# water-chika/ray-tracing-gpu-vulkan

Measured on AMD Instinct MI355X. Metric: Msamples/s (1920x1080 RTIOW scene, depth 50), higher is better.
Workload: dtype f32; 1 GPU; rtiow-1920x1080-10000spp-depth50 (BASELINE config 3 workload); width=1920, height=1080, spp=10000, depth=50, spheres=488, accel=grid-lds-rec, walk=uniform grid (3D DDA) staged in LDS, with the winner's gate and shading records, structure_build=host (binned-SAH LBVH + uniform grid), uploaded per frame, rng=hash, sample_chunks=10, parallelism=1 GPU, frames_in_flight=1

## Files before the change

ray-tracing-gpu-vulkan_amd/csrc/rt_internal.h:

```cpp
#pragma once

#include <stdint.h>

#include "../../include/rt_abi.h"
#include "rt_hand_out.h"

namespace rt {

struct alignas(16) GeomRec {
    float cx, cy, cz, rr;
};

struct alignas(16) MatRec {
    float c0x, c0y, c0z, attr;
    float c1x, c1y, c1z;
    uint32_t type_tex;
};
constexpr uint32_t kMatDielConst = 1u << 16;

#if defined(__HIPCC__)
__host__ __device__
#endif
inline bool colours_in_unit(const Sphere& s) {
    auto in = [](float v) { return v >= 0.0f && v <= 1.0f; };
// ... 17 lines not shown
        m.c1x = ef;
        m.c1y = qf * qf;
        m.c1z = qb * qb;
        m.type_tex |= kMatDielConst;
    }
    return m;
}

struct alignas(16) BvhNode {
    float lox, loy, loz;
    uint32_t escape;
    float hix, hiy, hiz;
    uint32_t first_count;
};

struct GridInfo {
    float gmin[3];
    float gmax[3];
    float cs[3];
    float inv_cs[3];
    float margin;
    float lo_m[3];
    float hi_m[3];
    uint32_t n[3];
    uint32_t n_cells, n_refs;
};

#ifndef RT_TRACE_BLOCK
#define RT_TRACE_BLOCK 768
#endif
constexpr unsigned kLaneSumLdsBytes = 3u * 8u * RT_TRACE_BLOCK;
constexpr unsigned kCoopLdsBytes = (2u * 16u + 8u + 4u) * RT_TRACE_BLOCK;
constexpr unsigned kCqLdsBytes = (128u * 4u + 4u) * (RT_TRACE_BLOCK / 64u) + 8u * RT_TRACE_BLOCK;
constexpr unsigned kBatchQueue = 64u;
constexpr unsigned kBatchLdsBytes = (4u + 16u + 16u + 12u) * RT_TRACE_BLOCK;
constexpr uint32_t kBatchMaxDepth = 1u << 26;

struct DeviceScene {
    uint32_t n_spheres = 0;
    GeomRec* geom = nullptr;
    float* radius = nullptr;
    MatRec* mat = nullptr;
    uint32_t n_big = 0;
    uint32_t* big_ids = nullptr;
    uint32_t n_nodes = 0;
    BvhNode* nodes = nullptr;
    BvhNode* nodes_raw = nullptr;
    GeomRec* leaf_geom = nullptr;
    uint32_t* leaf_ids = nullptr;
    uint32_t n_leaf = 0;
    BvhNode* nodes_oct = nullptr;
    float* treelet = nullptr;
    uint32_t* treelet_count = nullptr;
    float small_rmax = 0.0f;
    float small_rmin = 0.0f;
    GridInfo grid{};
    uint32_t* cell_start = nullptr;
    GeomRec* grid_rec = nullptr;
    uint32_t* grid_ids = nullptr;
};

enum : uint32_t { ACCEL_BRUTE = 1, ACCEL_LBVH_GLOBAL = 2, ACCEL_LBVH_LDS = 3, ACCEL_LBVH_OCT = 4,
                  ACCEL_LBVH_TOP = 5, ACCEL_GRID = 6, ACCEL_GRID_GLOBAL = 7, ACCEL_GRID_COOP = 8,
                  ACCEL_GRID_GLOBAL_COOP = 9, ACCEL_GRID_REC = 10, ACCEL_GRID_CQ = 11, ACCEL_GRID_REC_CQ = 12,
                  ACCEL_COUNT = 13 };

enum : int { MODE_STREAM = 0, MODE_HASH = 1, MODE_PROBE = 2, MODE_FEATURES = 3, MODE_SCATTER = 4 };

// ... 73 lines not shown
    const GeomRec* grid_rec;
    const uint32_t* grid_ids;
    float* accum;
    uint32_t* out;
    unsigned long long* fixed;
    Counters* counters;
    const float* big_tab;
    const BlockEntry* block_tab;
    const TabSize* tab_size;
    const float* probe_rays;
    uint32_t* probe_out;
    float* feat0;
    float* feat1;
};

struct ScatterProbeParams {
    uint32_t n_spheres;
    const GeomRec* geom;
    const float* radius;
    const MatRec* mat;
    uint32_t n;
    const float* rays;
    const uint32_t* ids;
    const float* t;
    const uint32_t* seeds;
    uint32_t* out;
};

constexpr int kFixedFracBits = 24;
constexpr uint32_t kFixedFlush = 128;

constexpr uint32_t kBigMax = 64;
constexpr uint32_t kRecStatic = 512;
constexpr uint32_t kNoRowsLds = 0xffffffffu;
constexpr uint32_t kHashMaxSpp = 1u << 19;

}
```

ray-tracing-gpu-vulkan_amd/csrc/rt_kernels.hip:

```cpp
#include <hip/hip_runtime.h>

#include "rt_device_math.h"
#include "rt_internal.h"
#include "rt_launchers.h"
#include "rt_trace_diag.h"
#include "rt_trace_prims.h"
#include "rt_trace_units.h"
#include "rt_trace_shade.h"
#include "rt_trace_walk.h"
#include "rt_trace_grid_coop.h"
#include "rt_trace_batch.h"

using namespace rtd;

namespace {

#ifndef RT_BRUTE_WAVES_PER_SIMD
#define RT_BRUTE_WAVES_PER_SIMD 6
#endif
#ifndef RT_TRACE_WAVES_PER_SIMD
#define RT_TRACE_WAVES_PER_SIMD 6
#endif
constexpr uint32_t kBruteBlock = 256;
constexpr uint32_t kTraceBlock = RT_TRACE_BLOCK;
// ... 256 lines not shown
        const uint32_t n = min(P.n_spheres, rt::kRecStatic);
        for (uint32_t i = threadIdx.x; i < n; i += kTraceBlock) {
            const rt::GeomRec g = P.geom[i];
            s_rec[3 * i] = make_float4(g.cx, g.cy, g.cz, P.radius[i]);
            s_rec[3 * i + 1] = mat4[2 * i];
            s_rec[3 * i + 2] = mat4[2 * i + 1];
        }
        __syncthreads();
        lbvh_loop<COUNT, CQ ? LAYOUT_GRID_CQ : LAYOUT_GRID, MODE, true, FLAT, TAB>(P, reinterpret_cast<const float4*>(cst), lds,
                                                                              ids, s_rec, s_rec);
        return;
    }
    __syncthreads();
    lbvh_loop<COUNT, COOP ? LAYOUT_GRID_COOP : CQ ? LAYOUT_GRID_CQ : LAYOUT_GRID, MODE, false, FLAT, TAB>(P, reinterpret_cast<const float4*>(cst), lds, ids,
                                        reinterpret_cast<const float4*>(P.geom),
                                        reinterpret_cast<const float4*>(P.mat));
}

template <bool FLAT>
__global__ __launch_bounds__(kTraceBlock, RT_TRACE_WAVES_PER_SIMD) void rt_trace_grid_batch_kernel(const rt::TraceParams P) {
    UTIL_INIT;
    PLACEMENT_RECORD(P);
    extern __shared__ float4 lds[];
    const uint32_t nr = P.grid.n_refs, nc1 = P.grid.n_cells + 1u;
    const uint32_t n_id4 = (nr + 3u) / 4u;
    const float4* rec = reinterpret_cast<const float4*>(P.grid_rec);
    for (uint32_t i = threadIdx.x; i < nr; i += kTraceBlock) lds[i] = rec[i];
    uint32_t* ids = reinterpret_cast<uint32_t*>(lds + nr);
    for (uint32_t i = threadIdx.x; i < nr; i += kTraceBlock) ids[i] = P.grid_ids[i];
    uint32_t* cst = reinterpret_cast<uint32_t*>(lds + nr + n_id4);
    for (uint32_t i = threadIdx.x; i < nc1; i += kTraceBlock) cst[i] = P.cell_start[i];
    stage_walk_params(P, threadIdx.x);
    stage_rows(P, threadIdx.x, kTraceBlock);
    __syncthreads();
    batch_loop<FLAT>(P, reinterpret_cast<const float4*>(cst), lds, ids, reinterpret_cast<const float4*>(P.geom),
                     reinterpret_cast<const float4*>(P.mat));
    UTIL_FLUSH;
}

template <bool COUNT, int MODE, int TAB = 0>
__global__ __launch_bounds__(kTraceBlock, RT_TRACE_WAVES_PER_SIMD) void rt_trace_top_kernel(const rt::TraceParams P) {
    UTIL_INIT;
    PLACEMENT_RECORD(P);
    extern __shared__ float4 lds[];
    typedef const __attribute__((address_space(3))) float4* LdsF4;
    const uint32_t lbase = uint32_t(reinterpret_cast<uintptr_t>((LdsF4)lds));
    const uint32_t n_top = min(*P.treelet_count, rt::kTreeletCap);
    for (uint32_t i = threadIdx.x; i < n_top; i += kTraceBlock) {
        const float4* tl = reinterpret_cast<const float4*>(P.treelet);
        const float4 A = tl[2 * i], B = tl[2 * i + 1];
        const uint32_t miss = __float_as_uint(B.z), hit = __float_as_uint(B.w);
        lds[2 * i] = A;
        lds[2 * i + 1] = make_float4(B.x, B.y, __uint_as_float(miss == END ? END : lbase + miss * 32u),
                                     __uint_as_float(int32_t(hit) >= 0 ? lbase + hit * 32u : hit));
    }
    stage_walk_params(P, threadIdx.x);
    stage_rows(P, threadIdx.x, kTraceBlock);
    __syncthreads();
    lbvh_loop<COUNT, LAYOUT_TOP, MODE, false, false, TAB>(P, lds, reinterpret_cast<const float4*>(P.leaf_geom), P.leaf_ids,
                                       reinterpret_cast<const float4*>(P.geom),
                                       reinterpret_cast<const float4*>(P.mat));
}

}

namespace rt {
// ... 89 lines not shown
```

ray-tracing-gpu-vulkan_amd/csrc/rt_trace_batch.h:

```cpp
#pragma once

#include <hip/hip_runtime.h>
#include <stdint.h>

#include "rt_device_math.h"
#include "rt_internal.h"
#include "rt_trace_grid.h"
#include "rt_trace_prims.h"
#include "rt_trace_shade.h"
#include "rt_trace_units.h"
#include "rt_trace_walk.h"

using namespace rtd;

namespace {

__shared__ uint32_t s_pix_chain[RT_TRACE_BLOCK];
__shared__ float4 s_q_o[RT_TRACE_BLOCK];
__shared__ float4 s_q_d[RT_TRACE_BLOCK];
__shared__ float s_q_thr[3 * RT_TRACE_BLOCK];
static_assert(rt::kBatchQueue == 64u, "one queue slot per lane of a wave: slot = wave0 + entry");
static_assert(sizeof(s_pix_chain) + sizeof(s_q_o) + sizeof(s_q_d) + sizeof(s_q_thr) == rt::kBatchLdsBytes,
              "rt_internal.h");

__device__ __forceinline__ void batch_path_end(uint32_t wave0, uint32_t pix, const Path& t, uint32_t segs) {
    unsigned long long* s = s_lane_sum + wave0 + pix;
    __hip_atomic_fetch_add(s, (unsigned long long)t.qx, __ATOMIC_RELAXED, __HIP_MEMORY_SCOPE_WAVEFRONT);
    __hip_atomic_fetch_add(s + RT_TRACE_BLOCK, (unsigned long long)t.qy, __ATOMIC_RELAXED, __HIP_MEMORY_SCOPE_WAVEFRONT);
    __hip_atomic_fetch_add(s + 2 * RT_TRACE_BLOCK, (unsigned long long)t.qz, __ATOMIC_RELAXED,
                           __HIP_MEMORY_SCOPE_WAVEFRONT);
    __hip_atomic_fetch_add(s_pix_chain + wave0 + pix, segs, __ATOMIC_RELAXED, __HIP_MEMORY_SCOPE_WAVEFRONT);
}

template <bool FLAT>
__device__ __forceinline__ bool batch_segment(const rt::TraceParams& P, const Camera& cam,
                                              const float4* __restrict__ cst, const float4* __restrict__ refs,
                                              const uint32_t* __restrict__ ids, const float4* __restrict__ geom4,
                                              const float4* __restrict__ mat4, uint32_t lane, bool active, Ray& r,
                                              Path& t) {
    uint32_t n_box = 0, n_sph = 0, n_empty = 0;
    __builtin_amdgcn_s_setprio(1);
    setup_ray<false>(P, r);
    r.walk = true;
    if (active) walk<false, LAYOUT_GRID, FLAT>(P, cst, refs, ids, r, n_box, n_sph, n_empty);
    HitRec hr{};
    float rad = 0.0f;
    if (active && r.bi != 0xffffffffu) {
        hr = load_hit(geom4, mat4, r.bi);
        rad = P.radius[r.bi];
    }
    unsigned long long regate =
        __ballot(active && r.bi != 0xffffffffu && !aabb_hit(hr.g.x, hr.g.y, hr.g.z, rad, r.o, r.inv));
    if (P.force_regate) regate = __ballot(active);
    if (__builtin_expect(regate != 0ull, 0)) {
        regate_brute<false>(P, geom4, lane, regate, r);
        if (((regate >> lane) & 1ull) && r.bi != 0xffffffffu) hr = load_hit(geom4, mat4, r.bi);
    }
    __builtin_amdgcn_s_setprio(0);
    bool more = false, fresh = false;
    if (active) {
        t.s = 0u;
        t.s_end = 1u;
        t.qx = t.qy = t.qz = 0u;
        more = shade_rec<rt::MODE_HASH, true, true>(P, cam, hr, t, r.bi, r.best, r.o, r.d, fresh);
    }
    return more;
}

template <bool FLAT>
__device__ __forceinline__ void batch_loop(const rt::TraceParams& P, const float4* __restrict__ cst,
                                           const float4* __restrict__ refs, const uint32_t* __restrict__ ids,
                                           const float4* __restrict__ geom4, const float4* __restrict__ mat4) {
    const uint32_t lane = lane_id();
    const uint32_t wave0 = __builtin_amdgcn_readfirstlane(threadIdx.x & ~63u);
    const Camera cam = load_camera(P);
    {
        unsigned long long* z = s_lane_sum + wave0 + lane;
        z[0] = z[RT_TRACE_BLOCK] = z[2 * RT_TRACE_BLOCK] = 0ull;
        s_pix_chain[wave0 + lane] = 0u;
        lane_order();
    }
    uint32_t seg_w = 0, smp_w = 0;
    WaveBlock blk;
    first_block<0>(P, lane, blk);
    if (lane == 0) atomicMin(&P.counters->t_first, __builtin_amdgcn_s_memrealtime());
    bool have = blk.end != blk.next;
    auto take = [&]() -> bool {
        if (blk.dry) return false;
        uint32_t nb = 0u;
        if (lane == 0) nb = atomicAdd(&P.counters->work_head, 64u);
        nb = __builtin_amdgcn_readfirstlane(nb);
        if (nb >= P.n_units) {
            blk.dry = true;
            if (lane == 0) atomicMin(&P.counters->t_dry, __builtin_amdgcn_s_memrealtime());
            return false;
        }
        take_block(P, lane, blk, nb >> 6, block_tile(P, nb >> 6));
        return true;
    };
    if (!have) have = take();
    uint32_t s = blk.s0, qn = 0u, px = 0u, word = 0u;
    bool valid = false, live = false;
    Ray r{};
    r.d = v3(0.0f, 0.0f, 1.0f);
    Path t{};
    auto block_pixels = [&]() {
        const uint32_t lx = (blk.tile % P.tiles_x) * 8u + (lane & 7u);
        const uint32_t ly = (blk.tile / P.tiles_x) * 8u + (lane >> 3);
        valid = lx < P.band_w && ly < P.band_h;
        px = lx | (ly << 16);
        s = blk.s0;
    };
    if (have) block_pixels();
    while (have) {
        const unsigned long long idle = __ballot(!live);
        if (idle && qn) {
            const uint32_t n = min(uint32_t(__popcll(idle)), qn);
            const uint32_t rank = __builtin_amdgcn_mbcnt_hi(uint32_t(idle >> 32), __builtin_amdgcn_mbcnt_lo(uint32_t(idle), 0u));
            if (!live && rank < n) {
                const uint32_t e = wave0 + (qn - 1u - rank);
                const float4 a = s_q_o[e], b = s_q_d[e];
                r.o = v3(a.x, a.y, a.z);
                r.d = v3(b.x, b.y, b.z);
                t.seed = __float_as_uint(a.w);
                word = __float_as_uint(b.w);
                t.thr = v3(s_q_thr[e], s_q_thr[RT_TRACE_BLOCK + e], s_q_thr[2 * RT_TRACE_BLOCK + e]);
                live = true;
            }
            qn -= n;
            lane_order();
        }
        const unsigned long long tracing = __ballot(live);
        if (~tracing != 0ull && s < blk.s1) {
            Path c{};
            Ray rc{};
            rc.d = v3(0.0f, 0.0f, 1.0f);
            if (valid) {
                c.px = px;
                c.pixel_seed = blk.seed;
                c.s = s;
                V3 v;
                camera_ray<rt::MODE_HASH, true>(P, cam, c, rc.o, v);
                rc.d = normalize(v);
            }
            const bool more = batch_segment<FLAT>(P, cam, cst, refs, ids, geom4, mat4, lane, valid, rc, c);
            const uint32_t n_valid = __popcll(__ballot(valid));
            seg_w += n_valid;
            smp_w += n_valid;
            if (valid && !more) batch_path_end(wave0, lane, c, 1u);
            const unsigned long long surv = __ballot(valid && more);
            if (valid && more) {
                const uint32_t e = wave0 + __builtin_amdgcn_mbcnt_hi(uint32_t(surv >> 32), __builtin_amdgcn_mbcnt_lo(uint32_t(surv), 0u));
                s_q_o[e] = make_float4(rc.o.x, rc.o.y, rc.o.z, __uint_as_float(c.seed));
                s_q_d[e] = make_float4(rc.d.x, rc.d.y, rc.d.z, __uint_as_float(lane | (c.depth << 6)));
                s_q_thr[e] = c.thr.x;
                s_q_thr[RT_TRACE_BLOCK + e] = c.thr.y;
                s_q_thr[2 * RT_TRACE_BLOCK + e] = c.thr.z;
            }
            qn = __popcll(surv);
            lane_order();
            s++;
            continue;
        }
        if (!tracing) {
            lane_order();
            unsigned long long* z = s_lane_sum + wave0 + lane;
            const unsigned long long x = z[0], y = z[RT_TRACE_BLOCK], w = z[2 * RT_TRACE_BLOCK];
            const uint32_t chain = s_pix_chain[wave0 + lane];
            z[0] = z[RT_TRACE_BLOCK] = z[2 * RT_TRACE_BLOCK] = 0ull;
            s_pix_chain[wave0 + lane] = 0u;
            lane_order();
            if (valid) {
                Path f{};
                f.px = px;
                f.segs = chain;
                if (x | y | w) add_fixed(P, f, x, y, w);
                record_tile_cost<rt::MODE_HASH>(P, f);
            }
            have = take();
            if (have) block_pixels();
            continue;
        }
        seg_w += __popcll(tracing);
        t.depth = word >> 6;
        const bool more = batch_segment<FLAT>(P, cam, cst, refs, ids, geom4, mat4, lane, live, r, t);
        if (live) {
            if (more) {
                word = (word & 63u) | (t.depth << 6);
            } else {
                batch_path_end(wave0, word & 63u, t, (word >> 6) + 1u);
                live = false;
            }
        }
    }
    if (lane == 0) {
        atomicAdd(&P.counters->segments, (unsigned long long)seg_w);
        atomicAdd(&P.counters->samples, (unsigned long long)smp_w);
        atomicMax(&P.counters->t_last, __builtin_amdgcn_s_memrealtime());
    }
}

}
```

ray-tracing-gpu-vulkan_amd/csrc/rt_trace_grid.h:

```cpp
#pragma once

#include <hip/hip_runtime.h>
#include <stdint.h>

#include "rt_device_math.h"
#include "rt_internal.h"
#include "rt_trace_diag.h"
#include "rt_trace_prims.h"

using namespace rtd;

namespace {

template <bool COUNT, bool PAIRS, bool FLAT = false>
__device__ __forceinline__ void grid_walk(const rt::TraceParams& P, const uint32_t* __restrict__ cstart,
                                          const float4* __restrict__ rec, const uint32_t* __restrict__ ids,
                                          Ray& r, uint32_t& n_cell, uint32_t& n_sph, uint32_t& n_empty) {
    const float4 ex = s_walk_entry[0], ey = s_walk_entry[1], ez = s_walk_entry[2];
    const float4 axx = s_walk_axis[0], axy = s_walk_axis[1], axz = s_walk_axis[2];
    const float lo0 = ex.x, lo1 = ey.x, lo2 = ez.x, hi0 = ex.y, hi1 = ey.y, hi2 = ez.y;
    const float ics[3] = {ex.z, ey.z, ez.z}, gmn[3] = {axx.y, axy.y, axz.y}, csz[3] = {axx.x, axy.x, axz.x};
    const int nm1[3] = {int(__float_as_uint(ex.w)), int(__float_as_uint(ey.w)), int(__float_as_uint(ez.w))};
    const uint32_t n0 = __float_as_uint(axx.w), n1 = __float_as_uint(axy.w);
    const float x0 = (lo0 - r.o.x) * r.inv.x, x1 = (hi0 - r.o.x) * r.inv.x;
    const float y0 = (lo1 - r.o.y) * r.inv.y, y1 = (hi1 - r.o.y) * r.inv.y;
    const float z0 = (lo2 - r.o.z) * r.inv.z, z1 = (hi2 - r.o.z) * r.inv.z;
    const float tn = fmaxf(fmaxf(fmaxf(fminf(x0, x1), fminf(y0, y1)), fminf(z0, z1)), T_MIN);
    const float tf = fminf(fminf(fminf(fmaxf(x0, x1), fmaxf(y0, y1)), fmaxf(z0, z1)), r.limit);
    if (!(tn <= tf)) return;
    auto cell_of = [&](float p, int k) {
        const int c = int(floorf((p - gmn[k]) * ics[k]));
        return min(max(c, 0), nm1[k]);
    };
    int cx = cell_of(__builtin_fmaf(tn, r.d.x, r.o.x), 0);
    int cy = FLAT ? 0 : cell_of(__builtin_fmaf(tn, r.d.y, r.o.y), 1);
    int cz = cell_of(__builtin_fmaf(tn, r.d.z, r.o.z), 2);
    const int sx = r.d.x > 0.0f ? 1 : (r.d.x < 0.0f ? -1 : 0);
    const int sy = r.d.y > 0.0f ? 1 : (r.d.y < 0.0f ? -1 : 0);
    const int sz = r.d.z > 0.0f ? 1 : (r.d.z < 0.0f ? -1 : 0);
    auto bound_t = [&](int c, int s, int k, float o, float inv) {
        const float plane = __builtin_fmaf(float(c + (s > 0 ? 1 : 0)), csz[k], gmn[k]);
        return s == 0 ? __builtin_inff() : (plane - o) * inv;
    };
    float tx = bound_t(cx, sx, 0, r.o.x, r.inv.x);
    float ty = bound_t(cy, sy, 1, r.o.y, r.inv.y);
    float tz = bound_t(cz, sz, 2, r.o.z, r.inv.z);
    uint32_t cell = FLAT ? uint32_t(cz) * n0 + uint32_t(cx) : (uint32_t(cz) * n1 + uint32_t(cy)) * n0 + uint32_t(cx);
    if constexpr (FLAT && PAIRS) {
        uint32_t b = cstart[cell], e = cstart[cell + 1];
        for (;;) {
            const float tm = fminf(fminf(tx, ty), tz);
            uint32_t ncell = cell;
            const bool more = dda_step_xz(tm, tx, ty, tz, cx, cz, sx, sz, ncell, r.o, r.inv);
            const uint32_t nb = cstart[ncell], ne = cstart[ncell + 1];
            if (COUNT) {
                n_cell++;
                n_empty += b == e ? 1u : 0u;
            }
            uint32_t j = b;
// ... 79 lines not shown
```

ray-tracing-gpu-vulkan_amd/csrc/rt_trace_prims.h:

```cpp
#pragma once

#include <hip/hip_runtime.h>
#include <stdint.h>

#include "rt_device_math.h"
#include "rt_internal.h"
#include "rt_trace_diag.h"

using namespace rtd;

namespace {

constexpr float T_MIN = 0.001f;
constexpr float T_MAX_SUCC = 0x1.388002p+13f;

__device__ __forceinline__ bool aabb_hit(float cx, float cy, float cz, float r, V3 o, V3 inv) {
    const float x0 = ((cx - r) - o.x) * inv.x, x1 = ((cx + r) - o.x) * inv.x;
    const float y0 = ((cy - r) - o.y) * inv.y, y1 = ((cy + r) - o.y) * inv.y;
    const float z0 = ((cz - r) - o.z) * inv.z, z1 = ((cz + r) - o.z) * inv.z;
    const float tnear = fmaxf(fmaxf(fmaxf(fminf(x0, x1), fminf(y0, y1)), fminf(z0, z1)), T_MIN);
    const float tfar = fminf(fminf(fminf(fmaxf(x0, x1), fmaxf(y0, y1)), fmaxf(z0, z1)), 10000.0f);
    return tnear <= tfar;
}

// ... 8 lines not shown
    if (D >= 0.0f) {
        const float sq = sqrt_cr(D);
        const float t1 = (-b - sq) * ia;
        const float t2 = (-b + sq) * ia;
        const float t = (t1 >= T_MIN) ? t1 : t2;
        if (t >= T_MIN && t < best && (!GATE || aabb_hit(cx, cy, cz, radius[id], o, inv))) {
            best = t;
            bi = id;
        }
    }
}

__device__ __forceinline__ bool behind(float b, float c) { return b >= 0x1p-60f && c >= 0.0f; }

typedef float f4v __attribute__((ext_vector_type(4)));
__device__ __forceinline__ float4 lds_reload(const float4* p) {
    const f4v v = *(const volatile __attribute__((address_space(3))) f4v*)(p);
    return make_float4(v.x, v.y, v.z, v.w);
}

__shared__ float4 s_walk_axis[3];
__shared__ float2 s_walk_slack;
__shared__ float4 s_walk_entry[3];
__device__ __forceinline__ void stage_walk_params(const rt::TraceParams& P, uint32_t tid) {
    if (tid < 3u) {
        const uint32_t stride = tid == 0u ? 1u : tid == 1u ? P.grid.n[0] : P.grid.n[0] * P.grid.n[1];
        s_walk_axis[tid] = make_float4(P.grid.cs[tid], P.grid.gmin[tid], __uint_as_float(stride),
                                       __uint_as_float(P.grid.n[tid]));
        s_walk_entry[tid] = make_float4(P.grid.lo_m[tid], P.grid.hi_m[tid], P.grid.inv_cs[tid],
                                        __uint_as_float(P.grid.n[tid] - 1u));
    }
    if (tid == 3u) s_walk_slack = make_float2(P.cull_near_abs, P.cull_abs);
}

__device__ __forceinline__ bool dda_step(float tm, float& tx, float& ty, float& tz, int& cx, int& cy, int& cz,
                                         int sx, int sy, int sz, uint32_t& cell, V3 o, V3 inv) {
    const bool mx = tx == tm, my = !mx && ty == tm, mz = !mx && !my;
    const float4 ax = s_walk_axis[mx ? 0 : my ? 1 : 2];
    const int s = mx ? sx : my ? sy : sz;
    const int c = (mx ? cx : my ? cy : cz) + s;
    if (uint32_t(c) >= __float_as_uint(ax.w)) return false;
    cx = mx ? c : cx;
    cy = my ? c : cy;
    cz = mz ? c : cz;
    cell = s > 0 ? cell + __float_as_uint(ax.z) : cell - __float_as_uint(ax.z);
    const float ok = mx ? o.x : my ? o.y : o.z, ik = mx ? inv.x : my ? inv.y : inv.z;
    const float tnew = (__builtin_fmaf(float(c + (s > 0 ? 1 : 0)), ax.x, ax.y) - ok) * ik;
    tx = mx ? tnew : tx;
    ty = my ? tnew : ty;
    tz = mz ? tnew : tz;
    return true;
}

__device__ __forceinline__ bool dda_step_xz(float tm, float& tx, float ty, float& tz, int& cx, int& cz, int sx,
                                            int sz, uint32_t& cell, V3 o, V3 inv) {
    const bool mx = tx == tm;
    if (!mx && ty == tm) return false;
    const float4 ax = s_walk_axis[mx ? 0 : 2];
    const int s = mx ? sx : sz;
    const int c = (mx ? cx : cz) + s;
    if (uint32_t(c) >= __float_as_uint(ax.w)) return false;
    cx = mx ? c : cx;
    cz = mx ? cz : c;
    cell = s > 0 ? cell + __float_as_uint(ax.z) : cell - __float_as_uint(ax.z);
    const float ok = mx ? o.x : o.z, ik = mx ? inv.x : inv.z;
    const float tnew = (__builtin_fmaf(float(c + (s > 0 ? 1 : 0)), ax.x, ax.y) - ok) * ik;
// ... 118 lines not shown
```

ray-tracing-gpu-vulkan_amd/csrc/rt_trace_shade.h:

```cpp
#pragma once

#include <hip/hip_runtime.h>
#include <stdint.h>

#include "rt_device_math.h"
#include "rt_internal.h"
#include "rt_trace_diag.h"
#include "rt_trace_units.h"

using namespace rtd;

namespace {

struct Camera { V3 lf, hor, ver, ulc, cup, crt; };

__device__ __forceinline__ Camera load_camera(const rt::TraceParams& P) {
    return Camera{v3(P.lf[0], P.lf[1], P.lf[2]), v3(P.hor[0], P.hor[1], P.hor[2]),
                  v3(P.ver[0], P.ver[1], P.ver[2]), v3(P.ulc[0], P.ulc[1], P.ulc[2]),
                  v3(P.cup[0], P.cup[1], P.cup[2]), v3(P.crt[0], P.crt[1], P.crt[2])};
}

template <int MODE, bool FAST = false>
__device__ __forceinline__ void camera_ray(const rt::TraceParams& P, const Camera& cam, Path& ps, V3& o, V3& v) {
    UTIL(7, true);
// ... 56 lines not shown
    d = normalize(v);
    return true;
}

template <int MODE, bool LSUM>
__device__ __forceinline__ void sample_end(const rt::TraceParams& P, Path& ps, const V3 col) {
    ps.s++;
    if (MODE == rt::MODE_HASH) {
        ps.qx += sample_fixed(col.x);
        ps.qy += sample_fixed(col.y);
        ps.qz += sample_fixed(col.z);
        if ((ps.s & (rt::kFixedFlush - 1u)) == 0u) flush_fixed<LSUM>(P, ps);
    } else {
        ps.sx += double(col.x);
        ps.sy += double(col.y);
        ps.sz += double(col.z);
    }
}

struct HitRec {
    float4 g, m0, m1;
};

__device__ __forceinline__ HitRec load_hit(const float4* __restrict__ geom4, const float4* __restrict__ mat4,
                                           uint32_t bi) {
    return HitRec{geom4[bi], mat4[2 * bi], mat4[2 * bi + 1]};
}

__shared__ float4 s_rec[3 * rt::kRecStatic];
__device__ __forceinline__ HitRec load_hit_rec(uint32_t bi) {
    return HitRec{s_rec[3 * bi], s_rec[3 * bi + 1], s_rec[3 * bi + 2]};
}

template <int MODE, bool LSUM, bool FAST = false>
__device__ __forceinline__ bool shade_rec(const rt::TraceParams& P, const Camera& cam, const HitRec& hr, Path& ps,
                                          uint32_t bi, float best, V3& o, V3& d, bool& fresh) {
    if constexpr (MODE == rt::MODE_PROBE) {
        const size_t i = size_t(ps.px >> 16) * P.band_w + (ps.px & 0xffffu);
        P.probe_out[2 * i] = bi;
        P.probe_out[2 * i + 1] = __float_as_uint(best);
        return false;
    }
    if constexpr (MODE == rt::MODE_FEATURES) {
        V3 alb = v3(0.7f, 0.8f, 1.0f), n = v3(0.0f, 0.0f, 0.0f);
        float depth = 0.0f, hit = 0.0f;
        if (bi != 0xffffffffu) {
            const V3 p = v3(__builtin_fmaf(best, d.x, o.x), __builtin_fmaf(best, d.y, o.y),
                            __builtin_fmaf(best, d.z, o.z));
            const float4 m0 = hr.m0, m1 = hr.m1;
            const uint32_t ttype = (__float_as_uint(m1.w) >> 8) & 0xffu;
            const V3 outward = normalize(sub(p, v3(hr.g.x, hr.g.y, hr.g.z)));
            const bool front = dot(d, outward) < 0.0f;
            n = front ? outward : neg(outward);
            alb = v3(m0.x, m0.y, m0.z);
            if (ttype == 1u && !checker_positive(p.x, p.y, p.z)) alb = v3(m1.x, m1.y, m1.z);
            depth = best;
            hit = 1.0f;
        }
        FeatPath& fp = feat_path(ps);
        fp.far += alb.x; fp.fag += alb.y; fp.fab += alb.z; fp.fah += hit;
        fp.fnx += n.x; fp.fny += n.y; fp.fnz += n.z; fp.fdz += depth;
        ps.s++;
        if (ps.s >= ps.s_end) return false;
        V3 v;
        camera_ray<rt::MODE_HASH, FAST>(P, cam, ps, o, v);
        d = normalize(v);
        fresh = true;
        return true;
    }
    V3 att;
    bool scatter = false;
    V3 sd = v3(0.0f, 0.0f, 0.0f);
    V3 p = o;
    UTIL(3, true);
    if (bi == 0xffffffffu) {
        att = v3(0.7f, 0.8f, 1.0f);
    } else {
        UTIL(10, true);
        p = v3(__builtin_fmaf(best, d.x, o.x), __builtin_fmaf(best, d.y, o.y),
               __builtin_fmaf(best, d.z, o.z));
        const float4 gc4 = hr.g;
        const float4 m0 = hr.m0;
        const float4 m1 = hr.m1;
        const uint32_t tt = __float_as_uint(m1.w);
        const uint32_t mtype = tt & 0xffu, ttype = (tt >> 8) & 0xffu;
        const V3 outward = normalize(sub(p, v3(gc4.x, gc4.y, gc4.z)));
        const bool front = dot(d, outward) < 0.0f;
        const V3 n = front ? outward : neg(outward);
        att = v3(m0.x, m0.y, m0.z);
        if (ttype == 1u && !checker_positive(p.x, p.y, p.z)) att = v3(m1.x, m1.y, m1.z);
        V3 ru = v3(0.0f, 0.0f, 0.0f);
        if (mtype < 2u) { UTIL(9, true); ru = random_unit_vector(ps.seed); }
        if (mtype == 0u) {
            UTIL(4, true);
            sd = add(n, ru);
            if (fabsf(sd.x) < 1e-8f && fabsf(sd.y) < 1e-8f && fabsf(sd.z) < 1e-8f) sd = n;
        } else if (mtype == 1u) {
            UTIL(5, true);
            const V3 refl = reflect(d, n);
            const V3 fuzz = scale(m0.w, ru);
            const V3 sc = normalize(add(refl, fuzz));
            if (dot(sc, n) > 0.0f) sd = sc;
        } else if (mtype == 2u) {
            UTIL(6, true);
            float eta, r;
            if (tt & rt::kMatDielConst) {
                eta = front ? m1.x : m0.w;
                r = front ? m1.y : m1.z;
            } else {
                eta = front ? (1.0f / m0.w) : m0.w;
                const float q = (1.0f - eta) / (1.0f + eta);
                r = q * q;
            }
            const float cos_t = dot(neg(d), n);
            bool refracts = false;
            if (eta * sqrt_cr(1.0f - cos_t * cos_t) <= 1.0f) {
                const float refl = r + (1.0f - r) * pow5(1.0f - cos_t);
                refracts = refl < rnd(ps.seed);
            }
            sd = refracts ? refract(d, n, eta) : reflect(d, n);
        }
        scatter = !(sd.x == 0.0f && sd.y == 0.0f && sd.z == 0.0f);
    }
// ... 47 lines not shown
```

ray-tracing-gpu-vulkan_amd/csrc/rt_trace_walk.h:

```cpp
#pragma once

#include <hip/hip_runtime.h>
#include <stdint.h>

#include "rt_device_math.h"
#include "rt_internal.h"
#include "rt_trace_diag.h"
#include "rt_trace_grid.h"
#include "rt_trace_grid_cq.h"
#include "rt_trace_prims.h"

using namespace rtd;

namespace {

constexpr uint32_t END = 0xffffffffu;

enum : int { LAYOUT_GLOBAL = 0, LAYOUT_LDS1 = 1, LAYOUT_OCT = 2, LAYOUT_TOP = 3, LAYOUT_GRID = 4, LAYOUT_GRID_L2 = 5,
             LAYOUT_GRID_COOP = 6, LAYOUT_GRID_CQ = 7 };

struct RayBox { V3 inv, oi; };

__device__ __forceinline__ float node_inv(float inv) {
    return __builtin_fabsf(inv) > 0x1p100f ? __builtin_copysignf(0x1p100f, inv) : inv;
// ... 25 lines not shown
}

__device__ __forceinline__ uint32_t octant(const V3 d) {
    return (__float_as_uint(d.x) >> 31) | ((__float_as_uint(d.y) >> 31) << 1) | ((__float_as_uint(d.z) >> 31) << 2);
}

__device__ __forceinline__ void big_group(Ray& r, const float (&sb)[16], const uint32_t (&ib)[4]) {
    float bk[4], Dk[4];
    uint32_t cand = 0u;
#pragma unroll
    for (int k = 0; k < 4; ++k) {
        const float rr = sb[4 * k + 3] * sb[4 * k + 3];
        const float ocx = r.o.x - sb[4 * k], ocy = r.o.y - sb[4 * k + 1], ocz = r.o.z - sb[4 * k + 2];
        bk[k] = __builtin_fmaf(ocz, r.d.z, __builtin_fmaf(ocy, r.d.y, ocx * r.d.x));
        const float c = __builtin_fmaf(ocz, ocz, __builtin_fmaf(ocy, ocy, ocx * ocx)) - rr;
        Dk[k] = __builtin_fmaf(bk[k], bk[k], -(r.a * c));
        cand |= (Dk[k] >= 0.0f && !behind(bk[k], c) ? 1u : 0u) << k;
    }
#pragma unroll
    for (int k = 0; k < 4; ++k) {
        if ((cand >> k) & 1u) {
            const float sq = sqrt_cr(Dk[k]);
            float t = (-bk[k] - sq) * r.ia;
            if (!(t >= T_MIN)) t = (-bk[k] + sq) * r.ia;
            const uint32_t id = ib[k];
            if ((t >= T_MIN) & (t <= r.best) & ((t < r.best) | (id < r.bi))) {
                r.best = t;
                r.bi = id;
            }
        }
    }
}

template <bool FAST = false>
__device__ __forceinline__ void setup_ray(const rt::TraceParams& P, Ray& r) {
    typedef const __attribute__((address_space(4))) float* ConstF;
    typedef const __attribute__((address_space(4))) uint32_t* ConstU;
    const ConstF g = (ConstF)(P.big_tab);
    const ConstU gid = (ConstU)(P.big_tab + 4u * rt::kBigMax);
    float sb0[16];
    uint32_t ib0[4];
#pragma unroll
    for (uint32_t k = 0; k < 16; ++k) sb0[k] = g[k];
#pragma unroll
    for (uint32_t k = 0; k < 4; ++k) ib0[k] = gid[k];
    r.a = dot(r.d, r.d);
    r.ia = rcp_cr(r.a);
    r.inv = v3(rcp_cr(r.d.x), rcp_cr(r.d.y), rcp_cr(r.d.z));
    r.best = 10000.0f;
    r.bi = 0xffffffffu;
    big_group(r, sb0, ib0);
    for (uint32_t k0 = 4; !FAST && k0 < P.n_big; k0 += 4) {
        float sb[16];
        uint32_t ib[4];
#pragma unroll
        for (uint32_t k = 0; k < 16; ++k) sb[k] = g[k0 * 4u + k];
#pragma unroll
        for (uint32_t k = 0; k < 4; ++k) ib[k] = gid[k0 + k];
        big_group(r, sb, ib);
    }
    r.limit = cull_limit(P, r.best);
    r.walk = P.nodes != nullptr || P.cell_start != nullptr;
}

template <bool COUNT, bool LDS_LEAF>
__device__ __forceinline__ void leaf_test(const rt::TraceParams& P, const float4* __restrict__ leaf4,
                                          const uint32_t* __restrict__ leaf_ids, uint32_t first,
                                          uint32_t count, Ray& r, uint32_t& n_sph) {
    const float4 s0 = leaf4[first], s1 = leaf4[first + 1], s2 = leaf4[first + 2], s3 = leaf4[first + 3];
    test4(s0, s1, s2, s3, [&](uint32_t k) {
                       if (LDS_LEAF) return lds_reload(leaf4 + first + k);
                       const f4v v = *(const volatile __attribute__((address_space(1))) f4v*)(leaf4 + first + k);
                       return make_float4(v.x, v.y, v.z, v.w);
                   },
                    [&](uint32_t k) { return leaf_ids[first + k]; }, r.o, r.d, r.inv, r.a, r.ia, r.best,
                    r.bi, r.limit, P);
    if (COUNT) n_sph += count;
}

template <bool COUNT>
__device__ __forceinline__ void walk_global_range(const rt::TraceParams& P, const float4* __restrict__ gnodes,
                                                  const float4* __restrict__ leaf4,
                                                  const uint32_t* __restrict__ leaf_ids, const RayBox& q,
                                                  uint32_t gi, uint32_t bound, Ray& r, uint32_t& n_box,
// ... 23 lines not shown
    const float4 g = geom4[r.bi];
    return aabb_hit(g.x, g.y, g.z, REC ? g.w : P.radius[r.bi], r.o, r.inv);
}

template <bool COUNT>
__device__ __forceinline__ void regate_brute(const rt::TraceParams& P, const float4* __restrict__ geom4, uint32_t lane,
                                          unsigned long long need, Ray& r) {
    if (COUNT && lane == 0) atomicAdd(&P.counters->util[30], (unsigned long long)__popcll(need));
    while (need) {
        const int L = __ffsll(need) - 1;
        need &= need - 1ull;
        const V3 o = v3(__shfl(r.o.x, L), __shfl(r.o.y, L), __shfl(r.o.z, L));
        const V3 d = v3(__shfl(r.d.x, L), __shfl(r.d.y, L), __shfl(r.d.z, L));
        const V3 inv = v3(__shfl(r.inv.x, L), __shfl(r.inv.y, L), __shfl(r.inv.z, L));
        const float a = __shfl(r.a, L), ia = __shfl(r.ia, L);
        float best = T_MAX_SUCC;
        uint32_t bi = 0xffffffffu;
        for (uint32_t i = lane; i < P.n_spheres; i += 64u) {
            const float4 s = geom4[i];
            test_sphere(s.x, s.y, s.z, s.w, P.radius, o, d, inv, a, ia, i, best, bi);
        }
        unsigned long long key = (uint64_t(__float_as_uint(best)) << 32) | bi;
        for (int off = 32; off > 0; off >>= 1) {
            const unsigned long long k2 = __shfl_xor(key, off);
            key = k2 < key ? k2 : key;
        }
        if (int(lane) == L) {
            r.best = __uint_as_float(uint32_t(key >> 32));
            r.bi = uint32_t(key);
        }
    }
}

template <bool COUNT, int LAYOUT, bool FLAT = false>
__device__ __forceinline__ void walk(const rt::TraceParams& P, const float4* __restrict__ nodes4,
                                     const float4* __restrict__ leaf4, const uint32_t* __restrict__ leaf_ids,
                                     Ray& r, uint32_t& n_box, uint32_t& n_sph, uint32_t& n_empty) {
    if (LAYOUT == LAYOUT_GRID_CQ) {
        if (r.walk)
            grid_walk_cq<COUNT>(P, reinterpret_cast<const uint32_t*>(nodes4), leaf4, leaf_ids, r, n_box, n_sph, n_empty);
        return;
    }
    if (LAYOUT == LAYOUT_GRID || LAYOUT == LAYOUT_GRID_L2) {
        if (r.walk)
            grid_walk<COUNT, LAYOUT == LAYOUT_GRID_L2, FLAT>(P, reinterpret_cast<const uint32_t*>(nodes4), leaf4, leaf_ids,
                                                             r, n_box, n_sph, n_empty);
        return;
    }
    const RayBox q = ray_box(r.o, r.inv);
    typedef const __attribute__((address_space(3))) float4* LdsF4;
    if (LAYOUT == LAYOUT_GLOBAL) {
        walk_global_range<COUNT>(P, nodes4, leaf4, leaf_ids, q, r.walk ? 0u : P.n_nodes, P.n_nodes, r, n_box,
                                 n_sph);
    } else if (LAYOUT == LAYOUT_TOP) {
        const uint32_t nbase = uint32_t(reinterpret_cast<uintptr_t>((LdsF4)nodes4));
        const float4* gnodes = reinterpret_cast<const float4*>(P.nodes);
        uint32_t ni = r.walk ? nbase : END;
        for (;;) {
            uint32_t cont = END;
            while (int32_t(ni) >= 0) {
                UTIL(0, true);
                const float4 A = lds_f4(ni);
                const float4 B = lds_f4(ni + 16u);
                if (COUNT) n_box++;
                const bool hit = node_hit<1u>(A, B, q, r.limit);
                cont = __float_as_uint(B.z);
                ni = __float_as_uint(hit ? B.w : B.z);
            }
            const bool at = ni != END;
            if (!__ballot(at)) break;
            if (at) {
                UTIL(1, true);
                if (ni & 0x40000000u) {
                    const uint32_t g = ni & 0x3fffffffu;
                    const uint32_t eg = __float_as_uint(gnodes[2 * g].w);
                    walk_global_range<COUNT>(P, gnodes, leaf4, leaf_ids, q, g + 1u, eg == END ? P.n_nodes : eg, r,
                                             n_box, n_sph);
                } else {
// ... 41 lines not shown
```

Measured before the change: 21650 Msamples/s.

## Precompute camera-origin terms and stage gate records in LDS for batch kernel

For primary camera rays, per-ray setup now reads precomputed origin-relative terms from a small LDS table: the big-sphere oc and c values and the grid entry bounds minus the camera origin. This skips the big-sphere table loads and several subtractions per ray. Sphere centre plus radius gate records are staged in LDS, so hit loads fetch geometry from LDS instead of global. The queued throughput array is dropped in favour of packing the hit id and a checker-alternate bit into the queue word, with throughput re-read from the material table. The catch is that the packed-id path assumes queued rays have depth 1 and an id below 512, which is only checked when RT_BATCH_ASSERT is defined.

```diff
diff --git a/ray-tracing-gpu-vulkan_amd/csrc/rt_internal.h b/ray-tracing-gpu-vulkan_amd/csrc/rt_internal.h
--- a/ray-tracing-gpu-vulkan_amd/csrc/rt_internal.h
+++ b/ray-tracing-gpu-vulkan_amd/csrc/rt_internal.h
@@ -73,8 +73,21 @@
 constexpr unsigned kLaneSumLdsBytes = 3u * 8u * RT_TRACE_BLOCK;
 constexpr unsigned kCoopLdsBytes = (2u * 16u + 8u + 4u) * RT_TRACE_BLOCK;
 constexpr unsigned kCqLdsBytes = (128u * 4u + 4u) * (RT_TRACE_BLOCK / 64u) + 8u * RT_TRACE_BLOCK;
+#ifndef RT_BATCH_GATE_LDS
+#define RT_BATCH_GATE_LDS 1
+#endif
+#ifndef RT_BATCH_CAMERA_TERMS
+#define RT_BATCH_CAMERA_TERMS 1
+#endif
 constexpr unsigned kBatchQueue = 64u;
-constexpr unsigned kBatchLdsBytes = (4u + 16u + 16u + 12u) * RT_TRACE_BLOCK;
+constexpr unsigned kBatchGateRecs = 512u;
+constexpr unsigned kBatchCamTabBytes = 1024u;
+#if RT_BATCH_GATE_LDS
+constexpr unsigned kBatchLdsBytes = (4u + 16u + 16u) * RT_TRACE_BLOCK + 16u * kBatchGateRecs + kBatchCamTabBytes;
+#else
+constexpr unsigned kBatchLdsBytes =
+    (4u + 16u + 16u + 12u) * RT_TRACE_BLOCK + (RT_BATCH_CAMERA_TERMS ? kBatchCamTabBytes : 0u);
+#endif
 constexpr uint32_t kBatchMaxDepth = 1u << 26;
 
 struct DeviceScene {
@@ -214,6 +227,7 @@
 
 constexpr uint32_t kBigMax = 64;
 constexpr uint32_t kRecStatic = 512;
+static_assert(kBatchGateRecs == kRecStatic, "the camera-batch form runs where the REC form does: ids below kRecStatic");
 constexpr uint32_t kNoRowsLds = 0xffffffffu;
 constexpr uint32_t kHashMaxSpp = 1u << 19;
 
diff --git a/ray-tracing-gpu-vulkan_amd/csrc/rt_kernels.hip b/ray-tracing-gpu-vulkan_amd/csrc/rt_kernels.hip
--- a/ray-tracing-gpu-vulkan_amd/csrc/rt_kernels.hip
+++ b/ray-tracing-gpu-vulkan_amd/csrc/rt_kernels.hip
@@ -312,6 +312,8 @@
     for (uint32_t i = threadIdx.x; i < nc1; i += kTraceBlock) cst[i] = P.cell_start[i];
     stage_walk_params(P, threadIdx.x);
     stage_rows(P, threadIdx.x, kTraceBlock);
+    stage_gate(P, threadIdx.x, kTraceBlock);
+    stage_camera_terms(P, threadIdx.x);
     __syncthreads();
     batch_loop<FLAT>(P, reinterpret_cast<const float4*>(cst), lds, ids, reinterpret_cast<const float4*>(P.geom),
                      reinterpret_cast<const float4*>(P.mat));
diff --git a/ray-tracing-gpu-vulkan_amd/csrc/rt_trace_batch.h b/ray-tracing-gpu-vulkan_amd/csrc/rt_trace_batch.h
--- a/ray-tracing-gpu-vulkan_amd/csrc/rt_trace_batch.h
+++ b/ray-tracing-gpu-vulkan_amd/csrc/rt_trace_batch.h
@@ -1,5 +1,6 @@
 #pragma once
 
+#include <assert.h>
 #include <hip/hip_runtime.h>
 #include <stdint.h>
 
@@ -18,10 +19,42 @@
 __shared__ uint32_t s_pix_chain[RT_TRACE_BLOCK];
 __shared__ float4 s_q_o[RT_TRACE_BLOCK];
 __shared__ float4 s_q_d[RT_TRACE_BLOCK];
+static_assert(rt::kBatchQueue == 64u, "one queue slot per lane of a wave: slot = wave0 + entry");
+constexpr bool kGateLds = RT_BATCH_GATE_LDS != 0, kCameraTerms = RT_BATCH_CAMERA_TERMS != 0;
+#if RT_BATCH_GATE_LDS
+__shared__ float4 s_gate[rt::kBatchGateRecs + (RT_BATCH_CAMERA_TERMS ? 0u : rt::kBatchCamTabBytes / 16u)];
+static_assert(sizeof(s_pix_chain) + sizeof(s_q_o) + sizeof(s_q_d) + sizeof(s_gate) +
+                      (kCameraTerms ? sizeof(s_cam_tab) : 0u) == rt::kBatchLdsBytes, "rt_internal.h");
+static_assert(rt::kBatchLdsBytes == 36864u, "rt_launch.h kBatchStaticLdsBytes: 55 408 B, pinned by the plan's tests");
+#else
 __shared__ float s_q_thr[3 * RT_TRACE_BLOCK];
-static_assert(rt::kBatchQueue == 64u, "one queue slot per lane of a wave: slot = wave0 + entry");
-static_assert(sizeof(s_pix_chain) + sizeof(s_q_o) + sizeof(s_q_d) + sizeof(s_q_thr) == rt::kBatchLdsBytes,
-              "rt_internal.h");
+static_assert(sizeof(s_pix_chain) + sizeof(s_q_o) + sizeof(s_q_d) + sizeof(s_q_thr) +
+                      (kCameraTerms ? sizeof(s_cam_tab) : 0u) == rt::kBatchLdsBytes, "rt_internal.h");
+#endif
+
+__device__ __forceinline__ void stage_gate(const rt::TraceParams& P, uint32_t tid, uint32_t nthr) {
+#if RT_BATCH_GATE_LDS
+    const uint32_t n = min(P.n_spheres, rt::kBatchGateRecs);
+    for (uint32_t i = tid; i < n; i += nthr) {
+        const rt::GeomRec g = P.geom[i];
+        s_gate[i] = make_float4(g.cx, g.cy, g.cz, P.radius[i]);
+    }
+#endif
+}
+__device__ __forceinline__ void stage_camera_terms(const rt::TraceParams& P, uint32_t tid) {
+    if constexpr (!kCameraTerms) return;
+    if (tid < 4u) {
+        const float* sb = P.big_tab + 4u * tid;
+        const float rr = sb[3] * sb[3];
+        const float ocx = P.lf[0] - sb[0], ocy = P.lf[1] - sb[1], ocz = P.lf[2] - sb[2];
+        const float c = __builtin_fmaf(ocz, ocz, __builtin_fmaf(ocy, ocy, ocx * ocx)) - rr;
+        s_cam_tab[tid] = make_float4(ocx, ocy, ocz, c);
+    } else if (tid < 7u) {
+        const uint32_t k = tid - 4u;
+        s_cam_tab[tid] = make_float4(P.grid.lo_m[k] - P.lf[k], P.grid.hi_m[k] - P.lf[k], P.grid.inv_cs[k],
+                                     __uint_as_float(P.grid.n[k] - 1u));
+    }
+}
 
 __device__ __forceinline__ void batch_path_end(uint32_t wave0, uint32_t pix, const Path& t, uint32_t segs) {
     unsigned long long* s = s_lane_sum + wave0 + pix;
@@ -32,22 +65,32 @@
     __hip_atomic_fetch_add(s_pix_chain + wave0 + pix, segs, __ATOMIC_RELAXED, __HIP_MEMORY_SCOPE_WAVEFRONT);
 }
 
-template <bool FLAT>
+template <bool FLAT, bool CAMERA>
 __device__ __forceinline__ bool batch_segment(const rt::TraceParams& P, const Camera& cam,
                                               const float4* __restrict__ cst, const float4* __restrict__ refs,
                                               const uint32_t* __restrict__ ids, const float4* __restrict__ geom4,
                                               const float4* __restrict__ mat4, uint32_t lane, bool active, Ray& r,
-                                              Path& t) {
+                                              Path& t, uint32_t& alt) {
+    constexpr bool CAM = CAMERA && kCameraTerms;
     uint32_t n_box = 0, n_sph = 0, n_empty = 0;
     __builtin_amdgcn_s_setprio(1);
-    setup_ray<false>(P, r);
+    setup_ray<false, CAM>(P, r);
     r.walk = true;
-    if (active) walk<false, LAYOUT_GRID, FLAT>(P, cst, refs, ids, r, n_box, n_sph, n_empty);
+    if (active) walk<false, LAYOUT_GRID, FLAT, CAM>(P, cst, refs, ids, r, n_box, n_sph, n_empty);
     HitRec hr{};
     float rad = 0.0f;
     if (active && r.bi != 0xffffffffu) {
-        hr = load_hit(geom4, mat4, r.bi);
-        rad = P.radius[r.bi];
+        if constexpr (kGateLds) {
+            hr.m0 = mat4[2 * r.bi];
+            hr.m1 = mat4[2 * r.bi + 1];
+#if RT_BATCH_GATE_LDS
+            hr.g = s_gate[r.bi];
+#endif
+            rad = hr.g.w;
+        } else {
+            hr = load_hit(geom4, mat4, r.bi);
+            rad = P.radius[r.bi];
+        }
     }
     unsigned long long regate =
         __ballot(active && r.bi != 0xffffffffu && !aabb_hit(hr.g.x, hr.g.y, hr.g.z, rad, r.o, r.inv));
@@ -62,7 +105,12 @@
         t.s = 0u;
         t.s_end = 1u;
         t.qx = t.qy = t.qz = 0u;
-        more = shade_rec<rt::MODE_HASH, true, true>(P, cam, hr, t, r.bi, r.best, r.o, r.d, fresh);
+        if constexpr (CAMERA && kGateLds) {
+            alt = 0u;
+            more = shade_rec<rt::MODE_HASH, true, true, true>(P, cam, hr, t, r.bi, r.best, r.o, r.d, fresh, &alt);
+        } else {
+            more = shade_rec<rt::MODE_HASH, true, true>(P, cam, hr, t, r.bi, r.best, r.o, r.d, fresh);
+        }
     }
     return more;
 }
@@ -123,8 +171,15 @@
                 r.o = v3(a.x, a.y, a.z);
                 r.d = v3(b.x, b.y, b.z);
                 t.seed = __float_as_uint(a.w);
-                word = __float_as_uint(b.w);
+                const uint32_t w = __float_as_uint(b.w);
+#if RT_BATCH_GATE_LDS
+                const float4 m = mat4[w >> 6];
+                t.thr = v3(m.x, m.y, m.z);
+                word = (w & 63u) | (1u << 6);
+#else
+                word = w;
                 t.thr = v3(s_q_thr[e], s_q_thr[RT_TRACE_BLOCK + e], s_q_thr[2 * RT_TRACE_BLOCK + e]);
+#endif
                 live = true;
             }
             qn -= n;
@@ -143,7 +198,8 @@
                 camera_ray<rt::MODE_HASH, true>(P, cam, c, rc.o, v);
                 rc.d = normalize(v);
             }
-            const bool more = batch_segment<FLAT>(P, cam, cst, refs, ids, geom4, mat4, lane, valid, rc, c);
+            uint32_t alt = 0u;
+            const bool more = batch_segment<FLAT, true>(P, cam, cst, refs, ids, geom4, mat4, lane, valid, rc, c, alt);
             const uint32_t n_valid = __popcll(__ballot(valid));
             seg_w += n_valid;
             smp_w += n_valid;
@@ -152,10 +208,17 @@
             if (valid && more) {
                 const uint32_t e = wave0 + __builtin_amdgcn_mbcnt_hi(uint32_t(surv >> 32), __builtin_amdgcn_mbcnt_lo(uint32_t(surv), 0u));
                 s_q_o[e] = make_float4(rc.o.x, rc.o.y, rc.o.z, __uint_as_float(c.seed));
+#if RT_BATCH_GATE_LDS
+#ifdef RT_BATCH_ASSERT
+                assert(c.depth == 1u && rc.bi < rt::kBatchGateRecs);
+#endif
+                s_q_d[e] = make_float4(rc.d.x, rc.d.y, rc.d.z, __uint_as_float(lane | (alt << 6) | (rc.bi << 7)));
+#else
                 s_q_d[e] = make_float4(rc.d.x, rc.d.y, rc.d.z, __uint_as_float(lane | (c.depth << 6)));
                 s_q_thr[e] = c.thr.x;
                 s_q_thr[RT_TRACE_BLOCK + e] = c.thr.y;
                 s_q_thr[2 * RT_TRACE_BLOCK + e] = c.thr.z;
+#endif
             }
             qn = __popcll(surv);
             lane_order();
@@ -183,7 +246,8 @@
         }
         seg_w += __popcll(tracing);
         t.depth = word >> 6;
-        const bool more = batch_segment<FLAT>(P, cam, cst, refs, ids, geom4, mat4, lane, live, r, t);
+        uint32_t unused = 0u;
+        const bool more = batch_segment<FLAT, false>(P, cam, cst, refs, ids, geom4, mat4, lane, live, r, t, unused);
         if (live) {
             if (more) {
                 word = (word & 63u) | (t.depth << 6);
diff --git a/ray-tracing-gpu-vulkan_amd/csrc/rt_trace_grid.h b/ray-tracing-gpu-vulkan_amd/csrc/rt_trace_grid.h
--- a/ray-tracing-gpu-vulkan_amd/csrc/rt_trace_grid.h
+++ b/ray-tracing-gpu-vulkan_amd/csrc/rt_trace_grid.h
@@ -12,19 +12,20 @@
 
 namespace {
 
-template <bool COUNT, bool PAIRS, bool FLAT = false>
+template <bool COUNT, bool PAIRS, bool FLAT = false, bool CAMERA = false>
 __device__ __forceinline__ void grid_walk(const rt::TraceParams& P, const uint32_t* __restrict__ cstart,
                                           const float4* __restrict__ rec, const uint32_t* __restrict__ ids,
                                           Ray& r, uint32_t& n_cell, uint32_t& n_sph, uint32_t& n_empty) {
-    const float4 ex = s_walk_entry[0], ey = s_walk_entry[1], ez = s_walk_entry[2];
+    const float4 ex = CAMERA ? s_cam_tab[4] : s_walk_entry[0], ey = CAMERA ? s_cam_tab[5] : s_walk_entry[1],
+                 ez = CAMERA ? s_cam_tab[6] : s_walk_entry[2];
     const float4 axx = s_walk_axis[0], axy = s_walk_axis[1], axz = s_walk_axis[2];
     const float lo0 = ex.x, lo1 = ey.x, lo2 = ez.x, hi0 = ex.y, hi1 = ey.y, hi2 = ez.y;
     const float ics[3] = {ex.z, ey.z, ez.z}, gmn[3] = {axx.y, axy.y, axz.y}, csz[3] = {axx.x, axy.x, axz.x};
     const int nm1[3] = {int(__float_as_uint(ex.w)), int(__float_as_uint(ey.w)), int(__float_as_uint(ez.w))};
     const uint32_t n0 = __float_as_uint(axx.w), n1 = __float_as_uint(axy.w);
-    const float x0 = (lo0 - r.o.x) * r.inv.x, x1 = (hi0 - r.o.x) * r.inv.x;
-    const float y0 = (lo1 - r.o.y) * r.inv.y, y1 = (hi1 - r.o.y) * r.inv.y;
-    const float z0 = (lo2 - r.o.z) * r.inv.z, z1 = (hi2 - r.o.z) * r.inv.z;
+    const float x0 = (CAMERA ? lo0 : lo0 - r.o.x) * r.inv.x, x1 = (CAMERA ? hi0 : hi0 - r.o.x) * r.inv.x;
+    const float y0 = (CAMERA ? lo1 : lo1 - r.o.y) * r.inv.y, y1 = (CAMERA ? hi1 : hi1 - r.o.y) * r.inv.y;
+    const float z0 = (CAMERA ? lo2 : lo2 - r.o.z) * r.inv.z, z1 = (CAMERA ? hi2 : hi2 - r.o.z) * r.inv.z;
     const float tn = fmaxf(fmaxf(fmaxf(fminf(x0, x1), fminf(y0, y1)), fminf(z0, z1)), T_MIN);
     const float tf = fminf(fminf(fminf(fmaxf(x0, x1), fmaxf(y0, y1)), fmaxf(z0, z1)), r.limit);
     if (!(tn <= tf)) return;
diff --git a/ray-tracing-gpu-vulkan_amd/csrc/rt_trace_prims.h b/ray-tracing-gpu-vulkan_amd/csrc/rt_trace_prims.h
--- a/ray-tracing-gpu-vulkan_amd/csrc/rt_trace_prims.h
+++ b/ray-tracing-gpu-vulkan_amd/csrc/rt_trace_prims.h
@@ -64,6 +64,8 @@
     }
     if (tid == 3u) s_walk_slack = make_float2(P.cull_near_abs, P.cull_abs);
 }
+
+__shared__ float4 s_cam_tab[rt::kBatchCamTabBytes / 16u];
 
 __device__ __forceinline__ bool dda_step(float tm, float& tx, float& ty, float& tz, int& cx, int& cy, int& cz,
                                          int sx, int sy, int sz, uint32_t& cell, V3 o, V3 inv) {
diff --git a/ray-tracing-gpu-vulkan_amd/csrc/rt_trace_shade.h b/ray-tracing-gpu-vulkan_amd/csrc/rt_trace_shade.h
--- a/ray-tracing-gpu-vulkan_amd/csrc/rt_trace_shade.h
+++ b/ray-tracing-gpu-vulkan_amd/csrc/rt_trace_shade.h
@@ -112,9 +112,10 @@
     return HitRec{s_rec[3 * bi], s_rec[3 * bi + 1], s_rec[3 * bi + 2]};
 }
 
-template <int MODE, bool LSUM, bool FAST = false>
+template <int MODE, bool LSUM, bool FAST = false, bool ALT = false>
 __device__ __forceinline__ bool shade_rec(const rt::TraceParams& P, const Camera& cam, const HitRec& hr, Path& ps,
-                                          uint32_t bi, float best, V3& o, V3& d, bool& fresh) {
+                                          uint32_t bi, float best, V3& o, V3& d, bool& fresh,
+                                          uint32_t* alt = nullptr) {
     if constexpr (MODE == rt::MODE_PROBE) {
         const size_t i = size_t(ps.px >> 16) * P.band_w + (ps.px & 0xffffu);
         P.probe_out[2 * i] = bi;
@@ -168,7 +169,10 @@
         const bool front = dot(d, outward) < 0.0f;
         const V3 n = front ? outward : neg(outward);
         att = v3(m0.x, m0.y, m0.z);
-        if (ttype == 1u && !checker_positive(p.x, p.y, p.z)) att = v3(m1.x, m1.y, m1.z);
+        if (ttype == 1u && !checker_positive(p.x, p.y, p.z)) {
+            att = v3(m1.x, m1.y, m1.z);
+            if constexpr (ALT) *alt = 1u;
+        }
         V3 ru = v3(0.0f, 0.0f, 0.0f);
         if (mtype < 2u) { UTIL(9, true); ru = random_unit_vector(ps.seed); }
         if (mtype == 0u) {
diff --git a/ray-tracing-gpu-vulkan_amd/csrc/rt_trace_walk.h b/ray-tracing-gpu-vulkan_amd/csrc/rt_trace_walk.h
--- a/ray-tracing-gpu-vulkan_amd/csrc/rt_trace_walk.h
+++ b/ray-tracing-gpu-vulkan_amd/csrc/rt_trace_walk.h
@@ -81,7 +81,32 @@
     }
 }
 
-template <bool FAST = false>
+__device__ __forceinline__ void big_group_camera(Ray& r, const uint32_t (&ib)[4]) {
+    float bk[4], Dk[4];
+    uint32_t cand = 0u;
+#pragma unroll
+    for (int k = 0; k < 4; ++k) {
+        const float4 q = s_cam_tab[k];
+        bk[k] = __builtin_fmaf(q.z, r.d.z, __builtin_fmaf(q.y, r.d.y, q.x * r.d.x));
+        Dk[k] = __builtin_fmaf(bk[k], bk[k], -(r.a * q.w));
+        cand |= (Dk[k] >= 0.0f && !behind(bk[k], q.w) ? 1u : 0u) << k;
+    }
+#pragma unroll
+    for (int k = 0; k < 4; ++k) {
+        if ((cand >> k) & 1u) {
+            const float sq = sqrt_cr(Dk[k]);
+            float t = (-bk[k] - sq) * r.ia;
+            if (!(t >= T_MIN)) t = (-bk[k] + sq) * r.ia;
+            const uint32_t id = ib[k];
+            if ((t >= T_MIN) & (t <= r.best) & ((t < r.best) | (id < r.bi))) {
+                r.best = t;
+                r.bi = id;
+            }
+        }
+    }
+}
+
+template <bool FAST = false, bool CAMERA = false>
 __device__ __forceinline__ void setup_ray(const rt::TraceParams& P, Ray& r) {
     typedef const __attribute__((address_space(4))) float* ConstF;
     typedef const __attribute__((address_space(4))) uint32_t* ConstU;
@@ -89,8 +114,10 @@
     const ConstU gid = (ConstU)(P.big_tab + 4u * rt::kBigMax);
     float sb0[16];
     uint32_t ib0[4];
-#pragma unroll
-    for (uint32_t k = 0; k < 16; ++k) sb0[k] = g[k];
+    if constexpr (!CAMERA) {
+#pragma unroll
+        for (uint32_t k = 0; k < 16; ++k) sb0[k] = g[k];
+    }
 #pragma unroll
     for (uint32_t k = 0; k < 4; ++k) ib0[k] = gid[k];
     r.a = dot(r.d, r.d);
@@ -98,7 +125,8 @@
     r.inv = v3(rcp_cr(r.d.x), rcp_cr(r.d.y), rcp_cr(r.d.z));
     r.best = 10000.0f;
     r.bi = 0xffffffffu;
-    big_group(r, sb0, ib0);
+    if constexpr (CAMERA) big_group_camera(r, ib0);
+    else big_group(r, sb0, ib0);
     for (uint32_t k0 = 4; !FAST && k0 < P.n_big; k0 += 4) {
         float sb[16];
         uint32_t ib[4];
@@ -188,7 +216,7 @@
     }
 }
 
-template <bool COUNT, int LAYOUT, bool FLAT = false>
+template <bool COUNT, int LAYOUT, bool FLAT = false, bool CAMERA = false>
 __device__ __forceinline__ void walk(const rt::TraceParams& P, const float4* __restrict__ nodes4,
                                      const float4* __restrict__ leaf4, const uint32_t* __restrict__ leaf_ids,
                                      Ray& r, uint32_t& n_box, uint32_t& n_sph, uint32_t& n_empty) {
@@ -199,7 +227,7 @@
     }
     if (LAYOUT == LAYOUT_GRID || LAYOUT == LAYOUT_GRID_L2) {
         if (r.walk)
-            grid_walk<COUNT, LAYOUT == LAYOUT_GRID_L2, FLAT>(P, reinterpret_cast<const uint32_t*>(nodes4), leaf4, leaf_ids,
+            grid_walk<COUNT, LAYOUT == LAYOUT_GRID_L2, FLAT, CAMERA>(P, reinterpret_cast<const uint32_t*>(nodes4), leaf4, leaf_ids,
                                                              r, n_box, n_sph, n_empty);
         return;
     }
```

After: 21990 Msamples/s (median of 6 runs). 1.6% higher.
